# AIML-IfI/openset-imagenet

Hardware: AMD Instinct MI355X
Metric: images/sec (whole node) ResNet-50 + entropic-open-set, Protocol 2, 1/2/4/8 GPUs (higher is better)
Workload: dtype f32; 1 GPU; Protocol 2, ResNet-50, entropic open-set loss, batch 128/GPU; workload_key=p2, classes=30, batch_per_gpu=128, global_batch=128, image=3x224x224, loss=entropic, optimizer=adam lr=1e-3, parallelism=dp1

## Files before the change

openset-imagenet_amd/csrc/conv_wino.hip:

```cpp
#include "conv_common.h"
#include <algorithm>
#include <type_traits>
#include <utility>

using namespace osi_conv;

namespace {

#ifndef OSI_WABL
#define OSI_WABL 0
#endif
#ifndef OSI_FABL
#define OSI_FABL 0
#endif
#ifndef OSI_STAGE_OUT
#define OSI_STAGE_OUT 1
#endif
#ifndef OSI_XSPREAD
#define OSI_XSPREAD 8
#endif
constexpr int KC = 16;
constexpr int PF = 6;

struct WinoP {
    const float* x;
    const float* u;
    float* y;
    const float* sc;
    const float* sh;
    int H, W, Kc, Nc, TH, TW, T, KS, CB, MT, NT;
    int x_bytes, y_bytes, u_bytes;
    float* pmean;
    float* pm2;
    int P;
    float cnt, rcnt;
    const float* ey0;
    const float *escale0, *eshift0, *emean0, *einv0;
    float* esum;
    const float *osc, *osh;
    int orelu;
    int q, r, nfull;
    float* slab;
    int slab_bytes;
};

__device__ __forceinline__ f32x2 pk_add(f32x2 a, f32x2 b) {
    f32x2 r;
    asm volatile("v_pk_add_f32 %0, %1, %2" : "=v"(r) : "v"(a), "v"(b));
    return r;
}
__device__ __forceinline__ f32x2 pk_sub(f32x2 a, f32x2 b) {
    f32x2 r;
    asm volatile("v_pk_add_f32 %0, %1, %2 neg_lo:[0,1] neg_hi:[0,1]" : "=v"(r) : "v"(a), "v"(b));
    return r;
}
__device__ __forceinline__ f32x2 pk_neg(f32x2 a) {
    f32x2 r;
    asm volatile("v_pk_add_f32 %0, 0, %1 neg_lo:[0,1] neg_hi:[0,1]" : "=v"(r) : "v"(a));
    return r;
}
__device__ __forceinline__ f32x2 pk_fma(f32x2 a, f32x2 b, f32x2 c) {
    f32x2 r;
    asm volatile("v_pk_fma_f32 %0, %1, %2, %3" : "=v"(r) : "v"(a), "v"(b), "v"(c));
    return r;
}
__device__ __forceinline__ f32x4 pk_add(f32x4 a, f32x4 b) {
    const f32x2 lo = pk_add(__builtin_shufflevector(a, a, 0, 1), __builtin_shufflevector(b, b, 0, 1));
    const f32x2 hi = pk_add(__builtin_shufflevector(a, a, 2, 3), __builtin_shufflevector(b, b, 2, 3));
    return __builtin_shufflevector(lo, hi, 0, 1, 2, 3);
}
__device__ __forceinline__ f32x4 pk_sub(f32x4 a, f32x4 b) {
    const f32x2 lo = pk_sub(__builtin_shufflevector(a, a, 0, 1), __builtin_shufflevector(b, b, 0, 1));
    const f32x2 hi = pk_sub(__builtin_shufflevector(a, a, 2, 3), __builtin_shufflevector(b, b, 2, 3));
    return __builtin_shufflevector(lo, hi, 0, 1, 2, 3);
}

template <class F, int... I>
__device__ __forceinline__ void for_each_const(F& f, std::integer_sequence<int, I...>) {
    (f(std::integral_constant<int, I>{}), ...);
}

__device__ __forceinline__ float row16_sum(float v) {
    v += __builtin_bit_cast(float, __builtin_amdgcn_update_dpp(0, __builtin_bit_cast(int, v), 0xB1, 0xF, 0xF, true));
    v += __builtin_bit_cast(float, __builtin_amdgcn_update_dpp(0, __builtin_bit_cast(int, v), 0x4E, 0xF, 0xF, true));
    v += __builtin_bit_cast(float, __builtin_amdgcn_update_dpp(0, __builtin_bit_cast(int, v), 0x141, 0xF, 0xF, true));
    v += __builtin_bit_cast(float, __builtin_amdgcn_update_dpp(0, __builtin_bit_cast(int, v), 0x140, 0xF, 0xF, true));
    return v;
}

template <int FLIP>
__global__ __launch_bounds__(256) void k_wino_weights(const float* __restrict__ w, float* __restrict__ u, int Kc, int Nc, int KS, int CB) {
    const int idx = blockIdx.x * 256 + threadIdx.x;
    const int K4 = Kc / 4;
    if (idx >= K4 * Nc) return;
    const int n = idx % Nc, k0 = (idx / Nc) * 4;
    f32x4 g[3][3];
#pragma unroll
    for (int r = 0; r < 3; ++r)
#pragma unroll
        for (int s = 0; s < 3; ++s) {
            if (FLIP) {
#pragma unroll
                for (int e = 0; e < 4; ++e) g[r][s][e] = w[((size_t)((k0 + e) * 3 + (2 - r)) * 3 + (2 - s)) * Nc + n];
            } else g[r][s] = ld4(w + ((size_t)(n * 3 + r) * 3 + s) * Kc + k0);
        }
    f32x4 t[4][3];
#pragma unroll
    for (int s = 0; s < 3; ++s) {
        t[0][s] = g[0][s];
        t[1][s] = 0.5f * (g[0][s] + g[1][s] + g[2][s]);
        t[2][s] = 0.5f * (g[0][s] - g[1][s] + g[2][s]);
        t[3][s] = g[2][s];
    }
    const int ks = k0 / KC, j = (k0 % KC) / 8, h = (k0 % 8) / 4, cb = n / 32, lane = h * 32 + n % 32;
#pragma unroll
    for (int xi = 0; xi < 4; ++xi) {
        f32x4 v[4];
        v[0] = t[xi][0];
        v[1] = 0.5f * (t[xi][0] + t[xi][1] + t[xi][2]);
        v[2] = 0.5f * (t[xi][0] - t[xi][1] + t[xi][2]);
        v[3] = t[xi][2];
#pragma unroll
        for (int nu = 0; nu < 4; ++nu) {
            const int p = xi * 4 + nu;
            *reinterpret_cast<f32x4*>(u + ((((size_t)(p * KS + ks) * CB + cb) * 2 + j) * 64 + lane) * 4) = v[nu];
        }
    }
}

struct Seg { int v, ks0, ks1, slot; bool valid; };

__device__ __forceinline__ void unit_of(int v, int MT, int NT, int& mt, int& nt) {
    const int full = (MT / 8) * 8 * NT;
    if (v < full) {
        const int xcd = v & 7, slot = v >> 3;
        nt = slot % NT;
        mt = (slot / NT) * 8 + xcd;
    } else {
        const int rem = MT & 7, vv = v - full;
        mt = (MT / 8) * 8 + vv % rem;
        nt = vv / rem;
    }
}
__device__ __forceinline__ int piece_begin(int w, int r, int KS, int G) { return (int)(((long)w * r * KS) / G); }

__device__ __forceinline__ Seg seg_phase2(int w, int q, int r, int KS, int G, bool second, int first_u) {
    Seg s{0, 0, 0, -1, false};
    if (r == 0) return s;
    const int b0 = piece_begin(w, r, KS, G), b1 = piece_begin(w + 1, r, KS, G);
    if (b1 <= b0) return s;
    const int u0 = b0 / KS;
    if (!second) {
        s.v = q * G + u0; s.ks0 = b0 - u0 * KS; s.ks1 = min(KS, s.ks0 + (b1 - b0)); s.slot = 0; s.valid = true;
        return s;
    }
    if (b1 > (u0 + 1) * KS) { s.v = q * G + u0 + 1; s.ks0 = 0; s.ks1 = b1 - (u0 + 1) * KS; s.slot = 1; s.valid = true; }
    return s;
}
__device__ __forceinline__ Seg seg_first(int w, int nfull, int q, int r, int KS, int G) {
    if (w < nfull) return Seg{w, 0, KS, -1, true};
    return seg_phase2(w, q, r, KS, G, false, 0);
}
__device__ __forceinline__ Seg seg_next(const Seg& c, int w, int nfull, int q, int r, int KS, int G) {
    if (c.slot < 0) {
        if (c.v + G < nfull) return Seg{c.v + G, 0, KS, -1, true};
        return seg_phase2(w, q, r, KS, G, false, 0);
    }
    if (c.slot == 0) return seg_phase2(w, q, r, KS, G, true, 0);
    return Seg{0, 0, 0, -1, false};
}

template <bool ODD, class PUT>
__device__ __forceinline__ void epi0_quad(const WinoP& p, PUT put, int g, f32x4 (&o)[4], const uint32_t (&po)[4], int ch0,
// ... 183 lines not shown
        }
    };

    f32x4 sc4 = {1, 1, 1, 1}, sh4 = {0, 0, 0, 0};
    load_x(seg.ks0);
    ld_scale(seg.ks0, sc4, sh4);
#pragma unroll
    for (int j = 0; j < 4; ++j) act_col(j, sc4, sh4);
#pragma unroll
    for (int i = 0; i < 4; ++i) row_store(i, 0);

    f32x4 a[16][2];
    auto load_u = [&](int pos, uint32_t base, int ks) {
        const uint32_t soff = (OSI_FABL & 1) ? 0u : (uint32_t)(pos * p.KS + ks) * ustep;
        a[pos][0] = bld4(ru, base, soff);
        a[pos][1] = bld4(ru, base + 1024u, soff);
    };
#pragma unroll
    for (int i = 0; i < PF; ++i) load_u(i, ua, seg.ks0);
    __syncthreads();

    int buf = 0;
    for (;;) {
#pragma unroll
        for (int i = 0; i < 16; ++i)
#pragma unroll
            for (int r = 0; r < 16; ++r) acc[i][r] = 0.f;
        Seg nxt{0, 0, 0, -1, false};
        const int cur_mt = mt, cur_nt = nt;
        for (int ks = seg.ks0; ks < seg.ks1; ++ks) {
            const bool last = ks + 1 == seg.ks1;
            int ksn = ks + 1;
            uint32_t uan = ua;
            if (last) {
                nxt = seg_next(seg, wg, p.nfull, p.q, p.r, p.KS, G);
                if (nxt.valid) unit_of(nxt.v, p.MT, p.NT, mt, nt);
                setup(mt, nt, nxt.valid, po_next, ua_next);
                ksn = nxt.valid ? nxt.ks0 : 0;
                uan = nxt.valid ? ua_next : ua;
            }
#if !(OSI_FABL & 2) && !OSI_XSPREAD
            load_x(ksn);
#endif
            ld_scale(ksn, sc4, sh4);
            const float* r0 = rb0 + buf * (16 * TB * KC);
            const float* r1 = rb1 + buf * (16 * TB * KC);
            f32x4 b0 = *reinterpret_cast<const f32x4*>(r0), b1 = *reinterpret_cast<const f32x4*>(r1);
            __builtin_amdgcn_sched_barrier(0);
            auto position = [&](auto POSC) {
                constexpr int pos = decltype(POSC)::value;
                if (pos + PF < 16) load_u(pos + PF, ua, ks);
                else load_u(pos + PF - 16, uan, ksn);
#if OSI_XSPREAD && !(OSI_FABL & 2)
                if constexpr (pos < OSI_XSPREAD) {
                    constexpr int n0 = pos * 16 / OSI_XSPREAD, n1 = (pos + 1) * 16 / OSI_XSPREAD;
#pragma unroll
                    for (int k = n0; k < n1; ++k) load_x1(ksn, k);
                }
#endif
                f32x4 nb0 = b0, nb1 = b1;
                if (pos < 15 && !(OSI_FABL & 8)) {
                    nb0 = *reinterpret_cast<const f32x4*>(r0 + (pos + 1) * (TB * KC));
                    nb1 = *reinterpret_cast<const f32x4*>(r1 + (pos + 1) * (TB * KC));
                }
                const f32x4 a0 = a[pos][0], a1 = a[pos][1];
#pragma unroll
                for (int e = 0; e < 4; ++e) acc[pos] = __builtin_amdgcn_mfma_f32_32x32x2f32(a0[e], b0[e], acc[pos], 0, 0, 0);
#pragma unroll
                for (int e = 0; e < 4; ++e) acc[pos] = __builtin_amdgcn_mfma_f32_32x32x2f32(a1[e], b1[e], acc[pos], 0, 0, 0);
#if !(OSI_FABL & 4)
                if constexpr (pos >= 8 && pos < 12) act_col(pos - 8, sc4, sh4);
                if constexpr (pos >= 12) row_store(pos - 12, buf ^ 1);
#endif
                b0 = nb0; b1 = nb1;
                __builtin_amdgcn_sched_barrier(0);
            };
            for_each_const(position, std::make_integer_sequence<int, 16>{});
            __syncthreads();
            buf ^= 1;
        }

        const int ch0 = CW * cur_nt + 32 * wm + 4 * hh;
        const int part = cur_mt * (TB / 16) + 2 * wn + ((lane >> 4) & 1);
        const __amdgpu_buffer_rsrc_t rs = make_rsrc(p.slab, p.slab_bytes);
        const __amdgpu_buffer_rsrc_t r0y = make_rsrc(EPI == 1 ? p.ey0 : p.y, p.y_bytes);
        Epi1Ops L1{};
        if constexpr (EPI == 1) { if (seg.slot < 0) L1 = epi1_load(p, r0y, 0, po, ch0); }
        float* const stage = WIDE ? sV + 2 * 16 * TB * KC : sV + (buf ^ 1) * (16 * TB * KC);
        if (seg.slot < 0 && wm == 0 && hh == 0) {
#pragma unroll
            for (int k = 0; k < 4; ++k) sPo[ntile * 4 + k] = po[k];
        }
#pragma unroll
        for (int g = (OSI_FABL & 16) ? 3 : 0; g < 4; ++g) {
            f32x4 o[4];
#pragma unroll
            for (int e = 0; e < 4; ++e) {
                const int r = 4 * g + e;
                float s[2][4];
#pragma unroll
                for (int nu = 0; nu < 4; ++nu) {
                    float m0, m1, m2, m3;
                    asm volatile("v_accvgpr_read_b32 %0, %1" : "=v"(m0) : "a"(acc[nu][r]));
                    asm volatile("v_accvgpr_read_b32 %0, %1" : "=v"(m1) : "a"(acc[4 + nu][r]));
                    asm volatile("v_accvgpr_read_b32 %0, %1" : "=v"(m2) : "a"(acc[8 + nu][r]));
                    asm volatile("v_accvgpr_read_b32 %0, %1" : "=v"(m3) : "a"(acc[12 + nu][r]));
                    s[0][nu] = m0 + m1 + m2;
                    s[1][nu] = m1 - m2 - m3;
                }
#pragma unroll
                for (int i = 0; i < 2; ++i) {
                    o[i * 2][e] = s[i][0] + s[i][1] + s[i][2];
                    o[i * 2 + 1][e] = s[i][1] - s[i][2] - s[i][3];
                }
            }
            if (seg.slot < 0) {
                auto put = [&](int k, int gq, const f32x4& v) {
#if OSI_STAGE_OUT
                    const int chunk = (32 * wm + 8 * gq + 4 * hh) >> 2;
                    *reinterpret_cast<f32x4*>(stage + (ntile * 4 + k) * CW + 4 * (chunk ^ (ntile & 15))) = v;
#else
                    bst4(ry, v, po[k] == OOB ? OOB : po[k] + 32u * gq, 0);
#endif
                };
                if constexpr (EPI == 0) epi0_quad<ODD>(p, put, g, o, po, ch0, part, lane);
                else if constexpr (EPI == 2) epi2_quad(p, put, g, o, ld4(p.osc + ch0 + 8 * g), ld4(p.osh + ch0 + 8 * g));
                else {
                    const Epi1Ops Ln = epi1_load(p, r0y, g < 3 ? g + 1 : 3, po, ch0);
                    epi1_apply<ODD>(p, put, g, o, po, ch0, part, lane, L1);
                    L1 = Ln;
                }
            } else {
                const uint32_t so = (uint32_t)((wg * 2 + seg.slot) * 65536 + ((wave * 4 + g) * 4) * 1024 + lane * 16);
#pragma unroll
                for (int k = 0; k < 4; ++k) bst4(rs, o[k], so + (uint32_t)k * 1024u, 0);
            }
        }
        if (OSI_STAGE_OUT && seg.slot < 0) {
            __syncthreads();
            constexpr int CPR = CW / 4, NCH = TB * 4 * CPR;
#pragma unroll 4
            for (int it = 0; it < NCH / 256; ++it) {
                const int idx = it * 256 + tid, row = idx / CPR, chunk = idx % CPR;
                const f32x4 v = *reinterpret_cast<const f32x4*>(stage + row * CW + 4 * (chunk ^ ((row >> 2) & 15)));
                const uint32_t base = sPo[row];
                bst4(ry, v, base == OOB ? OOB : base + (uint32_t)chunk * 16u, 0);
            }
            __syncthreads();
        }
        if (!nxt.valid) break;
        seg = nxt;
#pragma unroll
        for (int k = 0; k < 4; ++k) po[k] = po_next[k];
        ua = ua_next;
    }
}

template <int EPI, bool ODD, bool WIDE>
__global__ __launch_bounds__(64) void k_wino_fixup(WinoP p, int G) {
    const int lane = threadIdx.x, u = blockIdx.x >> 4, wave = (blockIdx.x >> 2) & 3, g = blockIdx.x & 3;
    const int wm = WIDE ? wave : wave >> 1, wn = WIDE ? 0 : wave & 1;
    const int ntile = 32 * wn + (lane & 31), hh = lane >> 5;
    int mt, nt;
    unit_of(p.q * G + u, p.MT, p.NT, mt, nt);
    uint32_t po[4];
    out_offsets<WIDE>(p, mt, nt, ntile, wm, hh, true, po);
    const __amdgpu_buffer_rsrc_t ry = make_rsrc(p.y, p.y_bytes);
    const __amdgpu_buffer_rsrc_t rs = make_rsrc(p.slab, p.slab_bytes);
    const int s0 = u * p.KS, s1 = s0 + p.KS;
    int w = (int)(((long)s0 * G) / ((long)p.r * p.KS));
    w = w > 0 ? w - 1 : 0;
    while (piece_begin(w + 1, p.r, p.KS, G) <= s0) ++w;
    f32x4 o[4] = {{0.f, 0.f, 0.f, 0.f}, {0.f, 0.f, 0.f, 0.f}, {0.f, 0.f, 0.f, 0.f}, {0.f, 0.f, 0.f, 0.f}};
    int b0 = piece_begin(w, p.r, p.KS, G);
    for (int ww = w; ww < G && b0 < s1; ++ww) {
        const int b1 = piece_begin(ww + 1, p.r, p.KS, G);
        if (b1 > b0) {
            const int slot = (b0 / p.KS == u) ? 0 : 1;
            const uint32_t so = (uint32_t)((ww * 2 + slot) * 65536 + ((wave * 4 + g) * 4) * 1024 + lane * 16);
#pragma unroll
            for (int k = 0; k < 4; ++k) o[k] += bld4(rs, so + (uint32_t)k * 1024u, 0);
        }
        b0 = b1;
    }
    const int ch0 = (WIDE ? 128 : 64) * nt + 32 * wm + 4 * hh, part = mt * (WIDE ? 2 : 4) + 2 * wn + ((lane >> 4) & 1);
    auto put = [&](int k, int gq, const f32x4& v) { bst4(ry, v, po[k] == OOB ? OOB : po[k] + 32u * gq, 0); };
    if constexpr (EPI == 0) epi0_quad<ODD>(p, put, g, o, po, ch0, part, lane);
    else if constexpr (EPI == 2) epi2_quad(p, put, g, o, ld4(p.osc + ch0 + 8 * g), ld4(p.osh + ch0 + 8 * g));
    else {
        const Epi1Ops L = epi1_load(p, make_rsrc(p.ey0, p.y_bytes), g, po, ch0);
        epi1_apply<ODD>(p, put, g, o, po, ch0, part, lane, L);
    }
}

struct WgradP {
    const float* x;
    const float* dy;
    float* slab;
    const float* sc;
    const float* sh;
    int H, W, Cin, Cout, TH, TW, T;
    int CBn, S, steps;
    int x_bytes, dy_bytes;
    FastDiv dTHW, dTW;
};

template <bool XF>
__global__ __launch_bounds__(512) void k_wino_wgrad(WgradP p) {
    __shared__ __attribute__((aligned(16))) float sL[2 * 2 * 16 * 2 * 64 * 4];
    const int tid = threadIdx.x, lane = tid & 63, hh = lane >> 5, l31 = lane & 31;
    const int wave = __builtin_amdgcn_readfirstlane(tid >> 6);
    const int ph = wave >> 2, wm = (wave >> 1) & 1, wn = wave & 1;
    const int item = blockIdx.x;
    const int split = item % p.S, blk = item / p.S, cb = blk % p.CBn, kb = blk / p.CBn;
    const int lh = wave & 1, kq = wave >> 1;
    const uint32_t xlane = (uint32_t)((cb * 64 + lane) * 4), dlane = (uint32_t)((kb * 64 + lane) * 4);
    const int t_first = split * p.steps * 8;
    const __amdgpu_buffer_rsrc_t rx = make_rsrc(p.x, p.x_bytes);
    const __amdgpu_buffer_rsrc_t rd = make_rsrc(p.dy, p.dy_bytes);
    float sc = 1.f, sh = 0.f;
    if constexpr (XF) { sc = p.sc[cb * 64 + lane]; sh = p.sh[cb * 64 + lane]; }
    const int cin4 = p.Cin * 4, cout4 = p.Cout * 4;

    float rx_[2][16], rd_[2][4];
    unsigned okx_[2], okd_[2];
    uint32_t srb[4], scb[4], sdr[2], sdc[2];
    auto prep_step = [&](int st, auto SETC) {
        constexpr int set = decltype(SETC)::value;
        const int t_raw = t_first + st * 8 + wave;
        const bool live = t_raw < p.T;
        const uint32_t t = (uint32_t)(live ? t_raw : p.T - 1);
        const uint32_t b = fdiv(t, p.dTHW), rem = t - b * p.dTHW.d, th = fdiv(rem, p.dTW), tw = rem - th * p.dTW.d;
        const int y0 = 2 * (int)th - 1, x0 = 2 * (int)tw - 1;
        unsigned rok = 0, cok = 0;
#pragma unroll
        for (int i = 0; i < 4; ++i) {
            const int yy = y0 + i, xx = x0 + i;
            rok |= ((unsigned)yy < (unsigned)p.H) ? (1u << i) : 0u;
            cok |= ((unsigned)xx < (unsigned)p.W) ? (1u << i) : 0u;
            srb[i] = (uint32_t)((((int)b * p.H + min(max(yy, 0), p.H - 1)) * p.W) * cin4);
            scb[i] = (uint32_t)(min(max(xx, 0), p.W - 1) * cin4);
        }
        if (!live) rok = 0;
        unsigned ok = 0;
#pragma unroll
        for (int i = 0; i < 4; ++i) ok |= ((rok >> i) & 1u) ? (cok << (4 * i)) : 0u;
        okx_[set] = ok;
#pragma unroll
        for (int i = 0; i < 2; ++i) {
            sdr[i] = (uint32_t)(((int)b * p.H + min(y0 + 1 + i, p.H - 1)) * p.W) * (uint32_t)cout4;
            sdc[i] = (uint32_t)min(x0 + 1 + i, p.W - 1) * (uint32_t)cout4;
        }
        okd_[set] = (((rok >> 1) & 1u) ? ((cok >> 1) & 3u) : 0u) | (((rok >> 2) & 1u) ? (((cok >> 1) & 3u) << 2) : 0u);
    };
    auto issue_load = [&](auto NC, auto SETC) {
        constexpr int n = decltype(NC)::value, set = decltype(SETC)::value;
        if constexpr (n < 16)
            rx_[set][n] = __builtin_bit_cast(float, __builtin_amdgcn_raw_buffer_load_b32(rx, xlane, srb[n / 4] + scb[n % 4], 0));
        else
            rd_[set][n - 16] = __builtin_bit_cast(float, __builtin_amdgcn_raw_buffer_load_b32(rd, dlane, sdr[(n - 16) / 2] + sdc[(n - 16) % 2], 0));
    };
    auto load_step = [&](int st, auto SETC) {
        prep_step(st, SETC);
        auto one = [&](auto NC) { issue_load(NC, SETC); };
        for_each_const(one, std::make_integer_sequence<int, 20>{});
    };
    auto img = [&](int buf, int op, int pos, int h, int ch) { return sL + ((((buf * 2 + op) * 16 + pos) * 2 + h) * 64 + ch) * 4; };
    float tx[16], td[4];
    auto act = [&](auto SETC) {
        constexpr int set = decltype(SETC)::value;
#pragma unroll
        for (int k = 0; k < 16; ++k) {
            float v = rx_[set][k];
            if constexpr (XF) asm volatile("v_fma_f32 %0, %1, %2, %3\n\tv_max_f32 %0, 0, %0" : "=v"(v) : "v"(rx_[set][k]), "v"(sc), "v"(sh));
            tx[k] = ((okx_[set] >> k) & 1u) ? v : 0.f;
        }
#pragma unroll
        for (int k = 0; k < 4; ++k) td[k] = ((okd_[set] >> k) & 1u) ? rd_[set][k] : 0.f;
    };
    auto col_x = [&]() {
#pragma unroll
        for (int j = 0; j < 4; ++j) {
            const float d0 = tx[j], d1 = tx[4 + j], d2 = tx[8 + j], d3 = tx[12 + j];
            tx[j] = d0 - d2; tx[4 + j] = d1 + d2; tx[8 + j] = d2 - d1; tx[12 + j] = d1 - d3;
        }
    };
    auto row_store = [&](int i, int buf) {
        const float t0 = tx[i * 4], t1 = tx[i * 4 + 1], t2 = tx[i * 4 + 2], t3 = tx[i * 4 + 3];
        const float v[4] = {t0 - t2, t1 + t2, t2 - t1, t1 - t3};
        const float a = td[0], b = td[1], c = td[2], d = td[3];
        const float e0 = i == 0 ? a : i == 1 ? a + c : i == 2 ? a - c : 0.f - c;
        const float e1 = i == 0 ? b : i == 1 ? b + d : i == 2 ? b - d : 0.f - d;
        const float y[4] = {e0, e0 + e1, e0 - e1, 0.f - e1};
#pragma unroll
        for (int nu = 0; nu < 4; ++nu) {
            img(buf, 1, i * 4 + nu, lh, lane)[kq] = v[nu];
            img(buf, 0, i * 4 + nu, lh, lane)[kq] = y[nu];
        }
    };

    f32x16 acc[8];
#pragma unroll
    for (int i = 0; i < 8; ++i)
#pragma unroll
        for (int r = 0; r < 16; ++r) acc[i][r] = 0.f;

// ... 101 lines not shown
    if (ph == 0) finish(S0{}); else finish(S1{});
}

__global__ __launch_bounds__(256) void k_wino_wgrad_reduce(const float* __restrict__ slab, float* __restrict__ dw, int Cin, int Cout, int CBn, int S,
                                                           int SG) {
    __shared__ f32x4 part[256];
    const int per = 256 / SG;
    const int o = threadIdx.x % per, g = threadIdx.x / per;
    const int idx = blockIdx.x * per + o;
    const int C4 = Cin / 4, n = Cout * 9 * C4;
    f32x4 a = {0.f, 0.f, 0.f, 0.f};
    int k = 0, tap = 0, c4 = 0;
    if (idx < n) {
        c4 = idx % C4; tap = (idx / C4) % 9; k = idx / (C4 * 9);
        const int cb = (c4 * 4) / 64, kb = k / 64;
        const float* src = slab + (size_t)((kb * CBn + cb) * S) * (9 * 4096) + (size_t)(tap * 64 + (k & 63)) * 64 + ((c4 * 4) & 63);
        for (int s = g; s < S; s += SG) a += ld4(src + (size_t)s * (9 * 4096));
    }
    part[threadIdx.x] = a;
    __syncthreads();
    if (g == 0 && idx < n) {
        for (int j = 1; j < SG; ++j) a += part[j * per + o];
        *reinterpret_cast<f32x4*>(dw + ((size_t)k * 9 + tap) * Cin + c4 * 4) = a;
    }
}

int backward_exclusive_cus();
struct WgradPlan { int S, steps; size_t slab_floats; };
WgradPlan plan_wgrad_wino(const osi_conv_desc* d) {
    const int T = d->B * ((d->H + 1) / 2) * ((d->W + 1) / 2);
    const int blocks = (d->Cout / 64) * (d->Cin / 64);
    int G = backward_exclusive_cus();
    int S = G / blocks;
    if (S < 1) S = 1;
    const int max_s = (T + 63) / 64;
    if (S > max_s) S = max_s;
    const int per = (T + S - 1) / S;
    WgradPlan w;
    w.S = S; w.steps = (per + 7) / 8;
    w.slab_floats = (size_t)blocks * S * 9 * 4096;
    return w;
}

bool wino_shape(const osi_conv_desc* d) {
    return conv_desc_ok(d) && d->R == 3 && d->S == 3 && d->stride == 1 && d->pad == 1 && d->H == d->Ho && d->W == d->Wo && d->H >= 2 && d->W >= 2;
}

struct Geo { int TH, TW, T, MT, P; bool odd; float cnt; bool uniform; };
Geo geo_of(const osi_conv_desc* d) {
    Geo g{};
    g.TH = (d->H + 1) / 2; g.TW = (d->W + 1) / 2; g.T = d->B * g.TH * g.TW; g.MT = (g.T + 63) / 64; g.P = (g.T + 15) / 16;
    const bool even = d->H % 2 == 0 && d->W % 2 == 0;
    g.odd = !even || g.T % 64 != 0;
    const int thw = g.TH * g.TW;
    if (g.P == 1) { g.uniform = true; g.cnt = (float)((long)d->B * d->H * d->W); }
    else if (g.T % 16 == 0 && even) { g.uniform = true; g.cnt = 64.f; }
    else if (g.T % 16 == 0 && 16 % thw == 0) { g.uniform = true; g.cnt = (float)(16 / thw * d->H * d->W); }
    else { g.uniform = false; g.cnt = 64.f; }
    return g;
}

template <int FLIP>
int launch_weights(const float* w, float* u, int Kc, int Nc, hipStream_t st) {
    hipLaunchKernelGGL(k_wino_weights<FLIP>, dim3((unsigned)((Kc / 4 * Nc + 255) / 256)), dim3(256), 0, st, w, u, Kc, Nc, Kc / KC, Nc / 32);
    OSI_LAUNCH_CHECK();
    return OSI_OK;
}

bool wide_units(int Nc) { return g_osi_tuning.wino_wide && Nc % 128 == 0; }

WinoP make_wp(const osi_conv_desc* d, const Geo& g, int Kc, int Nc) {
    WinoP p{};
    const bool wide = wide_units(Nc);
    p.H = d->H; p.W = d->W; p.Kc = Kc; p.Nc = Nc; p.TH = g.TH; p.TW = g.TW; p.T = g.T; p.KS = Kc / KC; p.CB = Nc / 32;
    p.MT = wide ? (g.T + 31) / 32 : g.MT; p.NT = Nc / (wide ? 128 : 64);
    p.x_bytes = (int)((size_t)d->B * d->H * d->W * Kc * 4);
    p.y_bytes = (int)((size_t)d->B * d->H * d->W * Nc * 4);
    p.u_bytes = (int)((size_t)16 * Kc * Nc * 4);
    p.P = g.P; p.cnt = g.cnt; p.rcnt = 1.f / g.cnt;
    return p;
}

int backward_exclusive_cus() {
    if (g_osi_tuning.tail_cus > 0) return chip_cus();
    int res = 8 * g_osi_tuning.dp_reserved_cus;
    if (res > hw_cus() / 4) res = hw_cus() / 4;
    const int n = hw_cus() - res;
    return n < 8 ? 8 : n;
}
int wino_grid(bool backward) {
    int cus = backward ? backward_exclusive_cus() : chip_cus();
    if (cus > hw_cus()) cus = hw_cus();
    cus = cus / 8 * 8;
    return cus < 8 ? 8 : cus;
}
constexpr size_t SLOT_BYTES = 65536;
size_t u_bytes_of(const osi_conv_desc* d) { return ((size_t)16 * d->Cin * d->Cout * sizeof(float) + 255) / 256 * 256; }
size_t slab_bytes_of() { return (size_t)(hw_cus() / 8 * 8 < 8 ? 8 : hw_cus() / 8 * 8) * 2 * SLOT_BYTES; }

void plan_units(WinoP& p, void* slab, size_t slab_bytes, const osi_conv_desc* d, int G, bool input_gradient) {
    const int V = p.MT * p.NT;
    p.q = V / G; p.r = V - p.q * G; p.nfull = p.q * G;
    const bool heavy_tail = p.r > 0 && (double)(G - p.r) / (double)G / (double)(p.q + 1) >= 0.15;
    const int sk = g_osi_tuning.wino_streamk;
    const bool cut = sk == 1 || (sk == 2 && !input_gradient) || (sk == 3 && input_gradient);
    if (!cut || (p.KS <= 4 && !heavy_tail)) { p.nfull = V; p.r = 0; }
    p.slab = (float*)slab;
    p.slab_bytes = (int)std::min<size_t>(slab_bytes, (size_t)hw_cus() * 2 * SLOT_BYTES);
}

}

extern "C" {

int osi_conv_wino_eligible(const osi_conv_desc* d, int input_gradient) {
    if (!wino_shape(d)) return 0;
    const int Kc = input_gradient ? d->Cout : d->Cin, Nc = input_gradient ? d->Cin : d->Cout;
    if (Kc % KC || Nc % 64) return 0;
    const Geo g = geo_of(d);
    return (input_gradient || g.uniform) ? 1 : 0;
}

size_t osi_conv_wino_workspace(const osi_conv_desc* d) {
    if (!wino_shape(d)) return 0;
    return u_bytes_of(d) + slab_bytes_of();
}

static int fwd_wino_impl(const osi_conv_desc* d, const float* x, const float* in_scale, const float* in_shift, const float* w, float* u,
                         float* y, void* slab, size_t slab_bytes, float* pstats, size_t pstats_bytes, int* P, int* rows_per_block,
                         osi_stream_t stream, const osi_conv_epilogue* epi = nullptr) {
    OSI_REQUIRE(x && u && y && slab && osi_conv_wino_eligible(d, 0));
    OSI_REQUIRE(!epi || (epi->scale && epi->shift && !epi->residual && !in_scale && !pstats));
    OSI_REQUIRE((in_scale == nullptr) == (in_shift == nullptr));
    OSI_REQUIRE(slab_bytes >= slab_bytes_of());
    OSI_REQUIRE(!pstats || (P && rows_per_block));
    hipStream_t st = (hipStream_t)stream;
    const Geo g = geo_of(d);
    WinoP p = make_wp(d, g, d->Cin, d->Cout);
    p.x = x; p.u = u; p.y = y; p.sc = in_scale; p.sh = in_shift;
    if (epi) { p.osc = epi->scale; p.osh = epi->shift; p.orelu = epi->relu ? 1 : 0; }
    if (pstats) {
        OSI_REQUIRE(pstats_bytes >= (size_t)2 * g.P * d->Cout * sizeof(float));
        p.pmean = pstats; p.pm2 = pstats + (size_t)g.P * d->Cout;
        *P = g.P; *rows_per_block = (int)g.cnt;
    }
    if (w) { if (int e = launch_weights<0>(w, u, d->Cin, d->Cout, st)) return e; }
    const int G = wino_grid(false);
    OSI_REQUIRE(slab_bytes >= (size_t)G * 2 * SLOT_BYTES);
    plan_units(p, slab, slab_bytes, d, G, false);
    const dim3 grid((unsigned)G), blk(256);
    const bool wide = wide_units(d->Cout), odd = g.odd || (wide && g.T % 32 != 0);
    auto launch = [&](auto XFC, auto ODDC, auto WIDEC) {
        constexpr bool xf = decltype(XFC)::value, od = decltype(ODDC)::value, wd = decltype(WIDEC)::value;
        hipLaunchKernelGGL((k_wino<xf, 0, od, wd>), grid, blk, 0, st, p);
        if (hipGetLastError() != hipSuccess) return OSI_ERR_LAUNCH;
        if (p.r > 0) {
            hipLaunchKernelGGL((k_wino_fixup<0, od, wd>), dim3((unsigned)p.r * 16), dim3(64), 0, st, p, G);
            if (hipGetLastError() != hipSuccess) return OSI_ERR_LAUNCH;
        }
        return OSI_OK;
    };
    auto launch_epi = [&](auto ODDC, auto WIDEC) {
        constexpr bool od = decltype(ODDC)::value, wd = decltype(WIDEC)::value;
        hipLaunchKernelGGL((k_wino<false, 2, od, wd>), grid, blk, 0, st, p);
        if (hipGetLastError() != hipSuccess) return OSI_ERR_LAUNCH;
        if (p.r > 0) {
            hipLaunchKernelGGL((k_wino_fixup<2, od, wd>), dim3((unsigned)p.r * 16), dim3(64), 0, st, p, G);
            if (hipGetLastError() != hipSuccess) return OSI_ERR_LAUNCH;
        }
        return OSI_OK;
    };
    using T_ = std::true_type; using F_ = std::false_type;
    if (epi) {
        if (odd) return wide ? launch_epi(T_{}, T_{}) : launch_epi(T_{}, F_{});
        return wide ? launch_epi(F_{}, T_{}) : launch_epi(F_{}, F_{});
    }
    const int sel = (in_scale ? 4 : 0) | (odd ? 2 : 0) | (wide ? 1 : 0);
    switch (sel) {
        case 0: return launch(F_{}, F_{}, F_{});
        case 1: return launch(F_{}, F_{}, T_{});
        case 2: return launch(F_{}, T_{}, F_{});
        case 3: return launch(F_{}, T_{}, T_{});
        case 4: return launch(T_{}, F_{}, F_{});
        case 5: return launch(T_{}, F_{}, T_{});
        case 6: return launch(T_{}, T_{}, F_{});
        default: return launch(T_{}, T_{}, T_{});
    }
}

int osi_conv_fwd_wino(const osi_conv_desc* d, const float* x, const float* in_scale, const float* in_shift, const float* w, float* y,
                      void* ws, size_t ws_bytes, float* pstats, size_t pstats_bytes, int* P, int* rows_per_block, osi_stream_t stream) {
    OSI_REQUIRE(w && ws && wino_shape(d) && ws_bytes >= osi_conv_wino_workspace(d));
    return fwd_wino_impl(d, x, in_scale, in_shift, w, (float*)ws, y, (char*)ws + u_bytes_of(d), ws_bytes - u_bytes_of(d), pstats, pstats_bytes, P,
                         rows_per_block, stream);
}

size_t osi_conv_wino_weights_bytes(const osi_conv_desc* d) { return wino_shape(d) ? u_bytes_of(d) : 0; }
size_t osi_conv_wino_slab_bytes(void) { return slab_bytes_of(); }
int osi_conv_wino_transform_weights(const osi_conv_desc* d, const float* w, int input_gradient, float* u, size_t u_bytes, osi_stream_t stream) {
    OSI_REQUIRE(w && u && osi_conv_wino_eligible(d, input_gradient ? 1 : 0) && u_bytes >= u_bytes_of(d));
    return input_gradient ? launch_weights<1>(w, u, d->Cout, d->Cin, (hipStream_t)stream) : launch_weights<0>(w, u, d->Cin, d->Cout, (hipStream_t)stream);
}
int osi_conv_fwd_wino_pre(const osi_conv_desc* d, const float* x, const float* in_scale, const float* in_shift, const float* u, float* y,
                          void* slab, size_t slab_bytes, float* pstats, size_t pstats_bytes, int* P, int* rows_per_block, osi_stream_t stream) {
    return fwd_wino_impl(d, x, in_scale, in_shift, nullptr, const_cast<float*>(u), y, slab, slab_bytes, pstats, pstats_bytes, P, rows_per_block, stream);
}

int osi_conv_fwd_wino_epilogue_pre(const osi_conv_desc* d, const float* x, const float* u, float* out, const osi_conv_epilogue* e, void* slab,
                                   size_t slab_bytes, osi_stream_t stream) {
    OSI_REQUIRE(e);
    return fwd_wino_impl(d, x, nullptr, nullptr, nullptr, const_cast<float*>(u), out, slab, slab_bytes, nullptr, 0, nullptr, nullptr, stream, e);
}

static int dgrad_wino_impl(const osi_conv_desc* d, const float* dy, const float* w, float* u, float* dx, const osi_dgrad_fusion* f, void* slab,
                           size_t slab_bytes, int* P, osi_stream_t stream) {
    OSI_REQUIRE(dy && u && dx && slab && f && P && osi_conv_wino_eligible(d, 1));
    OSI_REQUIRE(!f->relu_mask && !f->y1 && !f->pool_idx && f->addend_stride != 2);
    OSI_REQUIRE(f->y0 && f->scale0 && f->shift0);
    OSI_REQUIRE(!f->partials || (f->mean0 && f->invstd0));
    OSI_REQUIRE(slab_bytes >= slab_bytes_of());
    hipStream_t st = (hipStream_t)stream;
    const Geo g = geo_of(d);
    WinoP p = make_wp(d, g, d->Cout, d->Cin);
    p.x = dy; p.u = u; p.y = dx;
    p.ey0 = f->y0; p.escale0 = f->scale0; p.eshift0 = f->shift0;
    p.emean0 = f->mean0 ? f->mean0 : f->scale0; p.einv0 = f->invstd0 ? f->invstd0 : f->scale0;
    if (f->partials) {
        OSI_REQUIRE(f->partials_bytes >= (size_t)3 * g.P * d->Cin * sizeof(float));
        p.esum = f->partials;
    }
    *P = g.P;
    if (w) { if (int e = launch_weights<1>(w, u, d->Cout, d->Cin, st)) return e; }
    const int G = wino_grid(true);
    OSI_REQUIRE(slab_bytes >= (size_t)G * 2 * SLOT_BYTES);
    plan_units(p, slab, slab_bytes, d, G, true);
    const dim3 grid((unsigned)G), blk(256);
    const bool wide = wide_units(d->Cin), odd = g.odd || (wide && g.T % 32 != 0);
    auto launch = [&](auto ODDC, auto WIDEC) {
        constexpr bool od = decltype(ODDC)::value, wd = decltype(WIDEC)::value;
        hipLaunchKernelGGL((k_wino<false, 1, od, wd>), grid, blk, 0, st, p);
        if (hipGetLastError() != hipSuccess) return OSI_ERR_LAUNCH;
        if (p.r > 0) {
            hipLaunchKernelGGL((k_wino_fixup<1, od, wd>), dim3((unsigned)p.r * 16), dim3(64), 0, st, p, G);
            if (hipGetLastError() != hipSuccess) return OSI_ERR_LAUNCH;
        }
        return OSI_OK;
    };
    using T_ = std::true_type; using F_ = std::false_type;
    if (odd) return wide ? launch(T_{}, T_{}) : launch(T_{}, F_{});
    return wide ? launch(F_{}, T_{}) : launch(F_{}, F_{});
}

int osi_conv_dgrad_fused_wino(const osi_conv_desc* d, const float* dy, const float* w, float* dx, const osi_dgrad_fusion* f, void* ws,
                              size_t ws_bytes, int* P, osi_stream_t stream) {
    OSI_REQUIRE(w && ws && wino_shape(d) && ws_bytes >= osi_conv_wino_workspace(d));
    return dgrad_wino_impl(d, dy, w, (float*)ws, dx, f, (char*)ws + u_bytes_of(d), ws_bytes - u_bytes_of(d), P, stream);
}
int osi_conv_dgrad_fused_wino_pre(const osi_conv_desc* d, const float* dy, const float* u, float* dx, const osi_dgrad_fusion* f, void* slab,
                                  size_t slab_bytes, int* P, osi_stream_t stream) {
    return dgrad_wino_impl(d, dy, nullptr, const_cast<float*>(u), dx, f, slab, slab_bytes, P, stream);
}

size_t osi_conv_wgrad_wino_workspace(const osi_conv_desc* d) {
    if (!wino_shape(d) || d->Cin % 64 || d->Cout % 64) return 0;
    return plan_wgrad_wino(d).slab_floats * sizeof(float);
}

int osi_conv_wgrad_wino(const osi_conv_desc* d, const float* dy, const float* x, const float* in_scale, const float* in_shift, float* dw,
                        void* ws, size_t ws_bytes, osi_stream_t stream) {
    OSI_REQUIRE(dy && x && dw && ws && wino_shape(d) && d->Cin % 64 == 0 && d->Cout % 64 == 0);
    OSI_REQUIRE((in_scale == nullptr) == (in_shift == nullptr));
    const WgradPlan w = plan_wgrad_wino(d);
    OSI_REQUIRE(ws_bytes >= w.slab_floats * sizeof(float));
    hipStream_t st = (hipStream_t)stream;
    WgradP p{};
    p.x = x; p.dy = dy; p.slab = (float*)ws; p.sc = in_scale; p.sh = in_shift;
    p.H = d->H; p.W = d->W; p.Cin = d->Cin; p.Cout = d->Cout; p.TH = (d->H + 1) / 2; p.TW = (d->W + 1) / 2; p.T = d->B * p.TH * p.TW;
    p.CBn = d->Cin / 64; p.S = w.S; p.steps = w.steps;
    p.dTHW = make_fastdiv((uint32_t)(p.TH * p.TW)); p.dTW = make_fastdiv((uint32_t)p.TW);
    p.x_bytes = (int)((size_t)d->B * d->H * d->W * d->Cin * 4);
    p.dy_bytes = (int)((size_t)d->B * d->H * d->W * d->Cout * 4);
    const dim3 grid((unsigned)((d->Cout / 64) * p.CBn * p.S)), blk(256);
    if (in_scale) hipLaunchKernelGGL((k_wino_wgrad<true>), grid, dim3(512), 0, st, p);
    else hipLaunchKernelGGL((k_wino_wgrad<false>), grid, dim3(512), 0, st, p);
    OSI_LAUNCH_CHECK();
    const int n = d->Cout * 9 * (d->Cin / 4);
    int SG = 1;
    while (SG * 2 <= p.S && SG < 16) SG *= 2;
    const int per = 256 / SG;
    hipLaunchKernelGGL(k_wino_wgrad_reduce, dim3((unsigned)((n + per - 1) / per)), blk, 0, st, (const float*)ws, dw, d->Cin, d->Cout, p.CBn, p.S, SG);
    OSI_LAUNCH_CHECK();
    return OSI_OK;
}

}
```

Baseline: 4463 images/sec.

## Add 512-thread Winograd kernel splitting transform positions across two wave groups

Adds k_wino2, a 512-thread variant of the Winograd conv kernel in which two groups of four waves each compute half of the eight transform positions. Partial output-transform sums are exchanged through shared memory before the epilogue. By default it is used only for the forward path with fused input activation (XF), no epilogue, and the non-odd, non-wide shape. The aim is more waves per tile to hide latency and raise MFMA utilisation, at the cost of an extra LDS exchange and synchronisation plus higher register and shared-memory pressure per block.

```diff
diff --git a/openset-imagenet_amd/csrc/conv_wino.hip b/openset-imagenet_amd/csrc/conv_wino.hip
--- a/openset-imagenet_amd/csrc/conv_wino.hip
+++ b/openset-imagenet_amd/csrc/conv_wino.hip
@@ -19,6 +19,11 @@
 #ifndef OSI_XSPREAD
 #define OSI_XSPREAD 8
 #endif
+#ifndef OSI_WINO_TWO_WAVES
+#define OSI_WINO_TWO_WAVES 1
+#endif
+template <bool XF, int EPI, bool ODD, bool WIDE>
+constexpr bool two_waves() { return OSI_WINO_TWO_WAVES == 2 || (OSI_WINO_TWO_WAVES == 1 && XF && EPI == 0 && !ODD && !WIDE); }
 constexpr int KC = 16;
 constexpr int PF = 6;
 
@@ -508,6 +513,278 @@
         seg = nxt;
 #pragma unroll
         for (int k = 0; k < 4; ++k) po[k] = po_next[k];
+        ua = ua_next;
+    }
+}
+
+template <bool XF, int EPI, bool ODD, bool WIDE>
+__global__ __launch_bounds__(512) void k_wino2(WinoP p) {
+    constexpr int TB = WIDE ? 32 : 64, CW = WIDE ? 128 : 64, NV = WIDE ? 1 : 2, VB = 16 * TB * KC, PF2 = 3;
+    constexpr uint32_t ROOB = 0xC0000000u;
+    __shared__ __attribute__((aligned(16))) float sV[2 * VB + (WIDE ? 16384 : 0)];
+    __shared__ uint32_t sPo[TB * 4];
+    const int tid = threadIdx.x, lane = tid & 63;
+    const int wave = __builtin_amdgcn_readfirstlane(tid >> 6), ph = wave >> 2, wm = WIDE ? wave & 3 : (wave >> 1) & 1, wn = WIDE ? 0 : wave & 1;
+    const __amdgpu_buffer_rsrc_t rx = make_rsrc(p.x, p.x_bytes);
+    const __amdgpu_buffer_rsrc_t ry = make_rsrc(p.y, p.y_bytes);
+    const __amdgpu_buffer_rsrc_t ru = make_rsrc(p.u, p.u_bytes);
+    const int G = gridDim.x, wg = blockIdx.x;
+    const int ltile = WIDE ? tid >> 4 : tid >> 3, c = WIDE ? tid & 15 : 2 * (tid & 7);
+    const int ntile = 32 * wn + (lane & 31), hh = lane >> 5;
+    const int THW = p.TH * p.TW;
+    const uint32_t kc4 = (uint32_t)p.Kc * 4;
+
+    Seg seg = seg_first(wg, p.nfull, p.q, p.r, p.KS, G);
+    if (!seg.valid) return;
+    int mt, nt;
+    unit_of(seg.v, p.MT, p.NT, mt, nt);
+
+    uint32_t ro[4];
+    uint32_t cb[3];
+    uint32_t okb = 0;
+    auto setup = [&](int mt_, bool live) {
+        {
+            const int t = mt_ * TB + ltile;
+            const int b = t / THW, rem = t - b * THW, th = rem / p.TW, tw = rem - th * p.TW;
+            const bool tl = live && t < p.T;
+            uint32_t cm = 0;
+#pragma unroll
+            for (int j = 0; j < 4; ++j) {
+                const bool ok = (unsigned)(2 * tw - 1 + j) < (unsigned)p.W;
+                cm |= ok ? (1u << j) : 0u;
+                if (j != 1) cb[j == 0 ? 0 : j - 1] = ok ? 0u : OOB;
+            }
+            uint32_t m = 0;
+#pragma unroll
+            for (int i = 0; i < 4; ++i) {
+                const int yy = 2 * th - 1 + i;
+                const bool ok = tl && (unsigned)yy < (unsigned)p.H;
+                ro[i] = ok ? (uint32_t)((((b * p.H + yy) * p.W + 2 * tw) * p.Kc + c) * 4) : ROOB;
+                m |= ok ? (cm << (4 * i)) : 0u;
+            }
+            if constexpr (XF) okb = m;
+        }
+    };
+    setup(mt, true);
+    const uint32_t ulane = (uint32_t)lane * 16;
+    auto ucb = [&](int nt_) { return (uint32_t)((CW / 32) * nt_ + wm) * 2048u; };
+    uint32_t ua = ucb(nt), ua_next = ua;
+    float* const wbase = sV + ltile * KC + 4 * ((c >> 2) ^ ((ltile >> 2) & 3)) + (c & 3);
+    const float* const rb0 = sV + (2 * ph) * (TB * KC) + ntile * KC + 4 * ((0 + hh) ^ ((ntile >> 2) & 3));
+    const float* const rb1 = sV + (2 * ph) * (TB * KC) + ntile * KC + 4 * ((2 + hh) ^ ((ntile >> 2) & 3));
+    const uint32_t ustep = (uint32_t)p.CB * 2048;
+    auto pos_of = [&](int l) { return 4 * (l >> 1) + 2 * ph + (l & 1); };
+
+    f32x16 acc[8];
+    using XT = std::conditional_t<WIDE, float, f32x2>;
+    XT xr[16];
+    auto load_x1 = [&](int ks, int k) {
+        const int i = k >> 2, j = k & 3;
+        auto colb = [&](int jj) { return XF && !WIDE ? (~okb << (31 - (4 + jj))) & OOB : cb[jj == 0 ? 0 : jj - 1]; };
+        const uint32_t voff = j == 1 ? ro[i] : j == 0 ? (ro[i] - kc4) | colb(0) : ro[i] | colb(j);
+        const uint32_t soff = (uint32_t)ks * (KC * 4) + (j >= 2 ? (uint32_t)(j - 1) * kc4 : 0u);
+        if constexpr (WIDE) xr[k] = __builtin_bit_cast(float, __builtin_amdgcn_raw_buffer_load_b32(rx, voff, soff, 0));
+        else xr[k] = __builtin_bit_cast(f32x2, __builtin_amdgcn_raw_buffer_load_b64(rx, voff, soff, 0));
+    };
+    auto act1 = [&](float v, float s, float h, int keep) {
+        asm volatile("v_fma_f32 %0, %0, %1, %2\n\tv_max_f32 %0, 0, %0" : "+v"(v) : "v"(s), "v"(h));
+        return __builtin_bit_cast(float, __builtin_bit_cast(int, v) & keep);
+    };
+    auto act_col = [&](int j, XT sc, XT sh) {
+        if constexpr (XF) {
+#pragma unroll
+            for (int i = 0; i < 4; ++i) {
+                const int keep = (int)(okb << (31 - (i * 4 + j))) >> 31;
+                if constexpr (WIDE) xr[i * 4 + j] = act1(xr[i * 4 + j], sc, sh, keep);
+                else { xr[i * 4 + j][0] = act1(xr[i * 4 + j][0], sc[0], sh[0], keep); xr[i * 4 + j][1] = act1(xr[i * 4 + j][1], sc[1], sh[1], keep); }
+            }
+        }
+        const XT d0 = xr[j], d1 = xr[4 + j], d2 = xr[8 + j], d3 = xr[12 + j];
+        xr[j] = d0 - d2; xr[4 + j] = d1 + d2; xr[8 + j] = d2 - d1; xr[12 + j] = d1 - d3;
+    };
+    auto row_store = [&](int i, int buf) {
+        float* w = wbase + buf * VB + (i * 4) * (TB * KC);
+        const XT t0 = xr[i * 4], t1 = xr[i * 4 + 1], t2 = xr[i * 4 + 2], t3 = xr[i * 4 + 3];
+        auto st = [&](int nu, XT v) { *reinterpret_cast<XT*>(w + nu * (TB * KC)) = v; };
+        st(0, t0 - t2); st(1, t1 + t2); st(2, t2 - t1); st(3, t1 - t3);
+    };
+    XT sc{}, sh{};
+    auto ld_scale = [&](int ks) {
+        if constexpr (XF) { sc = *reinterpret_cast<const XT*>(p.sc + ks * KC + c); sh = *reinterpret_cast<const XT*>(p.sh + ks * KC + c); }
+    };
+
+#pragma unroll
+    for (int k = 0; k < 16; ++k) load_x1(seg.ks0, k);
+    ld_scale(seg.ks0);
+#pragma unroll
+    for (int j = 0; j < 4; ++j) act_col(j, sc, sh);
+#pragma unroll
+    for (int i = 0; i < 4; ++i) row_store(i, 0);
+
+    f32x4 a[4][2];
+    auto load_u = [&](int slot, int l, uint32_t base, int ks) {
+        const uint32_t soff = (uint32_t)(pos_of(l) * p.KS + ks) * ustep + base;
+        a[slot][0] = bld4(ru, ulane, soff);
+        a[slot][1] = bld4(ru, ulane + 1024u, soff);
+    };
+#pragma unroll
+    for (int l = 0; l < PF2; ++l) load_u(l, l, ua, seg.ks0);
+    __syncthreads();
+
+    using S0 = std::integral_constant<int, 0>;
+    using S1 = std::integral_constant<int, 1>;
+    int buf = 0;
+    for (;;) {
+#pragma unroll
+        for (int i = 0; i < 8; ++i)
+#pragma unroll
+            for (int r = 0; r < 16; ++r) acc[i][r] = 0.f;
+        Seg nxt{0, 0, 0, -1, false};
+        const int cur_mt = mt, cur_nt = nt;
+        for (int ks = seg.ks0; ks < seg.ks1; ++ks) {
+            const bool last = ks + 1 == seg.ks1;
+            int ksn = ks + 1;
+            uint32_t uan = ua;
+            if (last) {
+                nxt = seg_next(seg, wg, p.nfull, p.q, p.r, p.KS, G);
+                if (nxt.valid) unit_of(nxt.v, p.MT, p.NT, mt, nt);
+                setup(mt, nxt.valid);
+                ua_next = ucb(nt);
+                ksn = nxt.valid ? nxt.ks0 : 0;
+                uan = nxt.valid ? ua_next : ua;
+            }
+            const float* r0 = rb0 + buf * VB;
+            const float* r1 = rb1 + buf * VB;
+            f32x4 b0 = *reinterpret_cast<const f32x4*>(r0), b1 = b0;
+            if constexpr (WIDE) b1 = *reinterpret_cast<const f32x4*>(r1);
+            __builtin_amdgcn_sched_barrier(0);
+            auto position = [&](auto LC) {
+                constexpr int l = decltype(LC)::value, tl = l + PF2;
+                if constexpr (tl < 8) load_u(tl & 3, tl, ua, ks);
+                else load_u((tl - 8) & 3, tl - 8, uan, ksn);
+                if constexpr (l == 3) ld_scale(ksn);
+                if constexpr (l < 4) {
+#pragma unroll
+                    for (int j = 0; j < 4; ++j) load_x1(ksn, l * 4 + j);
+                }
+                f32x4 nb0 = b0, nb1 = b1;
+                if constexpr (!WIDE) b1 = *reinterpret_cast<const f32x4*>(r1 + (4 * (l >> 1) + (l & 1)) * (TB * KC));
+                if constexpr (l < 7) {
+                    constexpr int nofs = (4 * ((l + 1) >> 1) + ((l + 1) & 1)) * (TB * KC);
+                    nb0 = *reinterpret_cast<const f32x4*>(r0 + nofs);
+                    if constexpr (WIDE) nb1 = *reinterpret_cast<const f32x4*>(r1 + nofs);
+                }
+                const f32x4 a0 = a[l & 3][0], a1 = a[l & 3][1];
+#pragma unroll
+                for (int e = 0; e < 4; ++e) acc[l] = __builtin_amdgcn_mfma_f32_32x32x2f32(a0[e], b0[e], acc[l], 0, 0, 0);
+#pragma unroll
+                for (int e = 0; e < 4; ++e) acc[l] = __builtin_amdgcn_mfma_f32_32x32x2f32(a1[e], b1[e], acc[l], 0, 0, 0);
+                if constexpr (l == 4 || l == 5) { act_col(2 * (l - 4), sc, sh); act_col(2 * (l - 4) + 1, sc, sh); }
+                if constexpr (l >= 6) { row_store(2 * (l - 6), buf ^ 1); row_store(2 * (l - 6) + 1, buf ^ 1); }
+                b0 = nb0;
+                if constexpr (WIDE) b1 = nb1;
+                __builtin_amdgcn_sched_barrier(0);
+            };
+            for_each_const(position, std::make_integer_sequence<int, 8>{});
+            __syncthreads();
+            buf ^= 1;
+        }
+
+        const int ch0 = CW * cur_nt + 32 * wm + 4 * hh;
+        const int part = cur_mt * (TB / 16) + 2 * wn + ((lane >> 4) & 1);
+        uint32_t po[4];
+        out_offsets<WIDE>(p, cur_mt, cur_nt, ntile, wm, hh, true, po);
+        const __amdgpu_buffer_rsrc_t rs = make_rsrc(p.slab, p.slab_bytes);
+        const __amdgpu_buffer_rsrc_t r0y = make_rsrc(EPI == 1 ? p.ey0 : p.y, p.y_bytes);
+        float* const stage = WIDE ? sV + 2 * VB : sV + (buf ^ 1) * VB;
+        f32x4* const X = reinterpret_cast<f32x4*>(stage);
+        auto sloc = [&](int r, int i, int d) {
+            const float m0 = acc[d][r], m1 = acc[2 + d][r], m2 = acc[4 + d][r], m3 = acc[6 + d][r];
+            return i == 0 ? m0 + m1 + m2 : m1 - m2 - m3;
+        };
+        auto give = [&](auto PHC) {
+            constexpr int PH = decltype(PHC)::value;
+#pragma unroll
+            for (int gl = 0; gl < 2; ++gl)
+#pragma unroll
+                for (int i = 0; i < 2; ++i)
+#pragma unroll
+                    for (int d = 0; d < 2; ++d) {
+                        f32x4 v;
+#pragma unroll
+                        for (int e = 0; e < 4; ++e) v[e] = sloc(4 * (2 * (1 - PH) + gl) + e, i, d);
+                        X[(wave * 8 + (gl * 2 + i) * 2 + d) * 64 + lane] = v;
+                    }
+        };
+        if (ph == 0) give(S0{}); else give(S1{});
+        __syncthreads();
+        f32x4 rcv[2][2][2];
+#pragma unroll
+        for (int gl = 0; gl < 2; ++gl)
+#pragma unroll
+            for (int i = 0; i < 2; ++i)
+#pragma unroll
+                for (int d = 0; d < 2; ++d) rcv[gl][i][d] = X[((wave ^ 4) * 8 + (gl * 2 + i) * 2 + d) * 64 + lane];
+        __syncthreads();
+        if (seg.slot < 0 && ph == 0 && wm == 0 && hh == 0) {
+#pragma unroll
+            for (int k = 0; k < 4; ++k) sPo[ntile * 4 + k] = po[k];
+        }
+        auto finish = [&](auto PHC) {
+            constexpr int PH = decltype(PHC)::value;
+#pragma unroll
+            for (int gl = 0; gl < 2; ++gl) {
+                const int g = 2 * PH + gl;
+                f32x4 o[4];
+#pragma unroll
+                for (int e = 0; e < 4; ++e) {
+                    float s[2][4];
+#pragma unroll
+                    for (int i = 0; i < 2; ++i)
+#pragma unroll
+                        for (int d = 0; d < 2; ++d) {
+                            s[i][2 * PH + d] = sloc(4 * g + e, i, d);
+                            s[i][2 * (1 - PH) + d] = rcv[gl][i][d][e];
+                        }
+#pragma unroll
+                    for (int i = 0; i < 2; ++i) {
+                        o[i * 2][e] = s[i][0] + s[i][1] + s[i][2];
+                        o[i * 2 + 1][e] = s[i][1] - s[i][2] - s[i][3];
+                    }
+                }
+                if (seg.slot < 0) {
+                    auto put = [&](int k, int gq, const f32x4& v) {
+                        const int chunk = (32 * wm + 8 * gq + 4 * hh) >> 2;
+                        *reinterpret_cast<f32x4*>(stage + (ntile * 4 + k) * CW + 4 * (chunk ^ (ntile & 15))) = v;
+                    };
+                    if constexpr (EPI == 0) epi0_quad<ODD>(p, put, g, o, po, ch0, part, lane);
+                    else if constexpr (EPI == 2) epi2_quad(p, put, g, o, ld4(p.osc + ch0 + 8 * g), ld4(p.osh + ch0 + 8 * g));
+                    else {
+                        const Epi1Ops L1 = epi1_load(p, r0y, g, po, ch0);
+                        epi1_apply<ODD>(p, put, g, o, po, ch0, part, lane, L1);
+                    }
+                } else {
+                    const uint32_t so = (uint32_t)((wg * 2 + seg.slot) * 65536 + (((WIDE ? wm : wm * 2 + wn) * 4 + g) * 4) * 1024 + lane * 16);
+#pragma unroll
+                    for (int k = 0; k < 4; ++k) bst4(rs, o[k], so + (uint32_t)k * 1024u, 0);
+                }
+            }
+        };
+        if (ph == 0) finish(S0{}); else finish(S1{});
+        if (seg.slot < 0) {
+            __syncthreads();
+            constexpr int CPR = CW / 4, NCH = TB * 4 * CPR;
+#pragma unroll 4
+            for (int it = 0; it < NCH / 512; ++it) {
+                const int idx = it * 512 + tid, row = idx / CPR, chunk = idx % CPR;
+                const f32x4 v = *reinterpret_cast<const f32x4*>(stage + row * CW + 4 * (chunk ^ ((row >> 2) & 15)));
+                const uint32_t base = sPo[row];
+                bst4(ry, v, base == OOB ? OOB : base + (uint32_t)chunk * 16u, 0);
+            }
+            __syncthreads();
+        }
+        if (!nxt.valid) break;
+        seg = nxt;
         ua = ua_next;
     }
 }
@@ -915,7 +1192,8 @@
     const bool wide = wide_units(d->Cout), odd = g.odd || (wide && g.T % 32 != 0);
     auto launch = [&](auto XFC, auto ODDC, auto WIDEC) {
         constexpr bool xf = decltype(XFC)::value, od = decltype(ODDC)::value, wd = decltype(WIDEC)::value;
-        hipLaunchKernelGGL((k_wino<xf, 0, od, wd>), grid, blk, 0, st, p);
+        if constexpr (two_waves<xf, 0, od, wd>()) hipLaunchKernelGGL((k_wino2<xf, 0, od, wd>), grid, dim3(512), 0, st, p);
+        else hipLaunchKernelGGL((k_wino<xf, 0, od, wd>), grid, blk, 0, st, p);
         if (hipGetLastError() != hipSuccess) return OSI_ERR_LAUNCH;
         if (p.r > 0) {
             hipLaunchKernelGGL((k_wino_fixup<0, od, wd>), dim3((unsigned)p.r * 16), dim3(64), 0, st, p, G);
@@ -925,7 +1203,8 @@
     };
     auto launch_epi = [&](auto ODDC, auto WIDEC) {
         constexpr bool od = decltype(ODDC)::value, wd = decltype(WIDEC)::value;
-        hipLaunchKernelGGL((k_wino<false, 2, od, wd>), grid, blk, 0, st, p);
+        if constexpr (two_waves<false, 2, od, wd>()) hipLaunchKernelGGL((k_wino2<false, 2, od, wd>), grid, dim3(512), 0, st, p);
+        else hipLaunchKernelGGL((k_wino<false, 2, od, wd>), grid, blk, 0, st, p);
         if (hipGetLastError() != hipSuccess) return OSI_ERR_LAUNCH;
         if (p.r > 0) {
             hipLaunchKernelGGL((k_wino_fixup<2, od, wd>), dim3((unsigned)p.r * 16), dim3(64), 0, st, p, G);
@@ -1001,7 +1280,8 @@
     const bool wide = wide_units(d->Cin), odd = g.odd || (wide && g.T % 32 != 0);
     auto launch = [&](auto ODDC, auto WIDEC) {
         constexpr bool od = decltype(ODDC)::value, wd = decltype(WIDEC)::value;
-        hipLaunchKernelGGL((k_wino<false, 1, od, wd>), grid, blk, 0, st, p);
+        if constexpr (two_waves<false, 1, od, wd>()) hipLaunchKernelGGL((k_wino2<false, 1, od, wd>), grid, dim3(512), 0, st, p);
+        else hipLaunchKernelGGL((k_wino<false, 1, od, wd>), grid, blk, 0, st, p);
         if (hipGetLastError() != hipSuccess) return OSI_ERR_LAUNCH;
         if (p.r > 0) {
             hipLaunchKernelGGL((k_wino_fixup<1, od, wd>), dim3((unsigned)p.r * 16), dim3(64), 0, st, p, G);
```

Result: no change. 4435 images/sec (-0.6%).
